# EternityJune25/ComoRAG

Hardware: AMD Instinct MI355X
Metric: top-k queries/sec (higher is better)
Workload: dtype bf16; 1 GPU; brute-force top-20 over 10000000 x 768 bf16 rows, batch 64, row-sharded over 1 GPU(s) (north_star target config); rows=10000000, dim=768, batch=64, k=20, query_batches_rotated=4, device=AMD Radeon Graphics (gfx950:sramecc+:xnack-), n_cu=256, repeats=1, exchange=none (1 shard)

## Files before the change

### comorag_amd/csrc/api.hip

```cpp
#include <hip/hip_runtime.h>

#include <algorithm>
#include <cmath>
#include <cstdarg>
#include <cstdio>
#include <cstdlib>
#include <cstring>
#include <chrono>
#include <atomic>
#include <climits>
#include <map>
#include <memory>
#include <mutex>
#include <shared_mutex>
#include <string>
#include <vector>

#include "../../include/comorag_hip.h"
#include "cmr_kernels.h"
#include "cmr_internal.h"
#include "index_state.h"
#include "search_plan.h"
#include "prefilter_host.h"

// ... 49 lines not shown
    {"sync_poll", OPT_FIELD(sync_poll), Option::any, 0, 0, 0, nullptr, nullptr},
    {"scan_fin_dense", OPT_FIELD(fin_dense), Option::clamp, 1, 1 << 16, 0, nullptr, nullptr},
    {"scan_fin_cap", OPT_FIELD(fin_cap), Option::oneof, 0, 128, 256, "scan_fin_cap must be 0, 128 or 256", nullptr},
    {"scan_fin_suppliers", OPT_FIELD(fin_suppliers), Option::clamp, 0, CMR_FIN_SLOTS / CMR_SCAN_WAVES, 0, nullptr, nullptr},
    {"scan_fin_spin", OPT_FIELD(fin_spin), Option::clamp, 0, 1000, 0, nullptr, nullptr},
    {"scan_fin_queries", OPT_FIELD(fin_max_q), Option::clamp, 1, CMR_FIN_MAX_QUERIES, 0, nullptr, nullptr},
    {"sample_div", OPT_FIELD(sample_div), Option::clamp, 2, LLONG_MAX, 0, nullptr, nullptr},
    {"sample_maxmul", OPT_FIELD(sample_maxmul), Option::clamp, 0, LLONG_MAX, 0, nullptr, nullptr},
    {"pipe_reserve_cus", OPT_FIELD(reserve_cus), Option::any, 0, 0, 0, nullptr, nullptr},
    {"pipe_slots", OPT_FIELD(pipe_slots), Option::any, 0, 0, 0, nullptr, nullptr},
    {"wide_mode", OPT_FIELD(wide_mode), Option::range, 0, 2, 0, "wide_mode must be 0 (default), 1 (register-resident kernel) or 2 (query-split grid)", nullptr},
    {"stream_nt", OPT_FIELD(stream_nt), Option::any, 0, 0, 0, nullptr, nullptr},
    {"pipe_dual_scan", OPT_FIELD(dual_scan), Option::any, 0, 0, 0, nullptr, nullptr},
    {"pipe_cu_mask", OPT_FIELD(cu_mask), Option::any, 0, 0, 0, nullptr, nullptr},
    {"exact_cand", OPT_FIELD(exact_cand), Option::range, 2, CMR_MAX_K, 0, "exact_cand must be in [2, " CMR_STR(CMR_MAX_K) "]", OPT_READ(i->exact_cand)},
    {"combine", [](cmr_index* i, long long v) { i->combine.store((int)v, std::memory_order_relaxed); }, Option::zero_or, 2, cmr_combine::kMaxWidth, 0,
     "combine must be 0 (off) or in [2, " CMR_STR(CMR_PPR_MAX_BATCH) "]", OPT_READ(i->combine.load(std::memory_order_relaxed))},
    {"combine_wait_us", [](cmr_index* i, long long v) { i->combine_wait_us.store(v, std::memory_order_relaxed); }, Option::clamp, 0, 10000000, 0, nullptr,
     OPT_READ(i->combine_wait_us.load(std::memory_order_relaxed))},
    {"prefilter", OPT_FIELD(prefilter), Option::range, -1, 2, 0, "prefilter must be -1 (auto), 0 (off), 1 (on) or 2 (on, the filter keeps every row)", OPT_READ(i->prefilter)},
    {"prefilter_rescore_wgs", OPT_FIELD(pf_rescore_wgs), Option::clamp, 0, 1024, 0, nullptr, nullptr},
    {"prefilter_tighten", OPT_FIELD(pf_tighten), Option::range, 0, 1, 0, "prefilter_tighten must be 0 or 1", OPT_READ(i->pf_tighten)},
    {"prefilter_pair_cap", OPT_FIELD(pf_pair_cap), Option::clamp, 0, 1 << 20, 0, nullptr, OPT_READ(i->pf_pair_cap)},
    {"prefilter_active", nullptr, Option::any, 0, 0, 0, nullptr, OPT_READ(i->prefilter_active)},
    {"prefilter_rows", nullptr, Option::any, 0, 0, 0, nullptr, OPT_READ(i->q8c.q8 ? i->q8c.rows : 0)},
    {"prefilter_bytes", nullptr, Option::any, 0, 0, 0, nullptr, OPT_READ((long long)i->q8c.bytes(i->dpad))},
    {"prefilter_candidates", nullptr, Option::any, 0, 0, 0, nullptr, OPT_READ(q8_read_counter(i, Q8Counter::candidates))},
    {"prefilter_pairs", nullptr, Option::any, 0, 0, 0, nullptr, OPT_READ(q8_read_counter(i, Q8Counter::pairs))},
    {"prefilter_pair_overflow", nullptr, Option::any, 0, 0, 0, nullptr, OPT_READ(q8_read_counter(i, Q8Counter::pair_overflow))},
    {"last_route", nullptr, Option::any, 0, 0, 0, nullptr, OPT_READ(i->last_route.load(std::memory_order_relaxed))},
    {"pipe_dual_scan_active", nullptr, Option::any, 0, 0, 0, nullptr, OPT_READ(i->dual_active)},
    {"pipe_dual_scan_wide_active", nullptr, Option::any, 0, 0, 0, nullptr, OPT_READ(i->dual_wide_active)},
    {"pipe_cu_mask_active", nullptr, Option::any, 0, 0, 0, nullptr, OPT_READ(i->pipe.last_masked)},
    {"pipe_scan_cus", nullptr, Option::any, 0, 0, 0, nullptr, OPT_READ(i->pipe.last_masked ? i->pipe.scan_cus : i->n_cu)},
    {"combine_batches", nullptr, Option::any, 0, 0, 0, nullptr, OPT_READ(i->combiner.batches())},
    {"combine_queries", nullptr, Option::any, 0, 0, 0, nullptr, OPT_READ(i->combiner.queries())},
    {"combine_max_width", nullptr, Option::any, 0, 0, 0, nullptr, OPT_READ(i->combiner.max_width())},
};
#undef OPT_FIELD
#undef OPT_READ

const Option* find_option(const char* name) {
    for (const Option& o : kOptions) if (strcmp(o.name, name) == 0) return &o;
    return nullptr;
}

int set_option(cmr_index* idx, const char* name, long long v) {
    const Option* o = find_option(name ? name : "");
    if (!o || !o->store) return fail(CMR_ERR_INVALID, "unknown option '%s'", name ? name : "");
    const bool refused = o->kind == Option::oneof ? (v != o->a && v != o->b && v != o->c) : o->kind == Option::range ? (v < o->a || v > o->b) : o->kind == Option::zero_or ? (v != 0 && (v < o->a || v > o->b)) : false;
    if (refused) return fail(CMR_ERR_INVALID, "%s", o->reject);
    if (o->kind == Option::clamp) v = std::max(o->a, std::min(v, o->b));
// ... 1555 lines not shown
```

### comorag_amd/csrc/cmr_kernels.h

```cpp
#pragma once
#include <hip/hip_runtime.h>
#include <stdint.h>

typedef unsigned long long u64;

struct CmrScanGeom {
    int dtype;
    int dpad;
    int ks;
    int nqt;
    int cap;
    int ring;
    int grid;
    int asm_ring;
    size_t lds;
    int stream_default_policy;
};

int cmr_scan_max_nqt(int dtype, int dpad);
bool cmr_scan_geom(CmrScanGeom* g);

struct CmrScanArgs {
    const void* corpus;
    const void* qfrag;
// ... 101 lines not shown
size_t cmr_exact_part_bytes(int nq, int kc);
hipError_t cmr_launch_exact_certify(int dtype, const float* shadow, int dim, long long nrows, long long id_base, const long long* tab, int nb,
                                    const float* q, int nq, const int64_t* cand_ids, const float* cand_sc, int kc, int k, const float* stats,
                                    void* part, int* arrive, int64_t* out_ids, float* out_scores, int* out_exact, hipStream_t s);

hipError_t cmr_launch_q8_quantise(int dtype, const void* corpus, int dpad, long long panel0, long long npanels, long long nrows, void* q8,
                                  float2* scales, float* stats, hipStream_t s);
hipError_t cmr_launch_q8_pack_queries(int dtype, const float* q, int nq, int dim, int dpad, int tiles, const float* stats, void* qpack,
                                      float4* qconst, hipStream_t s);
struct CmrQ8Args {
    int dtype, dpad, nqt, cap;
    int grid;
    int rescore_grid;
    const void* corpus;
    const void* q8;
    const float2* scales;
    const void* qfrag;
    const void* qpack;
    const float4* qconst;
    const u64* tau_init;
    long long nrows;
    int npanels, nq, k;
    int keep_all;
    void* pair;
    unsigned* pair_cnt;
    int pcap;
    unsigned* keep;
    float* tau_tight;
    unsigned* cand_row;
    unsigned* n_cand;
    u64* lists;
    int* cnt;
};
hipError_t cmr_launch_q8_filter(const CmrQ8Args& a, hipStream_t s);
hipError_t cmr_launch_q8_tighten(const CmrQ8Args& a, hipStream_t s);
hipError_t cmr_launch_q8_expand(const CmrQ8Args& a, hipStream_t s);
hipError_t cmr_launch_q8_rescore(const CmrQ8Args& a, hipStream_t s);
int cmr_q8_rescore_waves(void);
```

### comorag_amd/csrc/index_state.h

```cpp
#pragma once
#include <hip/hip_runtime.h>

#include <algorithm>
#include <atomic>
#include <cstring>
#include <map>
#include <mutex>
#include <shared_mutex>
#include <vector>

#include "../../include/comorag_hip.h"
#include "cmr_kernels.h"
#include "cmr_internal.h"
#include "combine.h"

#define CMR_DT_F32 0
#define CMR_PANEL_ROWS 32
#define CMR_SCAN_WAVES 8
#define CMR_CORPUS_SLACK (128 * 1024)

namespace {

int elem_size(int dtype) { return dtype == CMR_F32 ? 4 : 2; }
int round_up(int x, int m) { return (x + m - 1) / m * m; }
long long panels_of(long long rows) { return (rows + CMR_PANEL_ROWS - 1) / CMR_PANEL_ROWS; }

struct ExactScratch {
    DevBuf ids, sc, part, arrive, oids, osc, oex;
    void release() { ids.release(); sc.release(); part.release(); arrive.release(); oids.release(); osc.release(); oex.release(); }
};

struct Q8Companion {
    void* q8 = nullptr; float2* scales = nullptr; float* stats = nullptr;
    long long cap_panels = 0, rows = 0;
    long long failed_cap = -1;
    hipEvent_t ready = nullptr; hipStream_t stream = nullptr;
    size_t bytes(int dpad) const { return q8 ? (size_t)cap_panels * CMR_PANEL_ROWS * (dpad + sizeof(float2)) + CMR_CORPUS_SLACK : 0; }
    void release() { (void)hipFree(q8); (void)hipFree(scales); (void)hipFree(stats); if (ready) (void)hipEventDestroy(ready); *this = Q8Companion{}; }
};
enum Q8Buf { Q8_QPACK, Q8_QCONST, Q8_CAND, Q8_NCAND, Q8_PAIR, Q8_PAIRCNT, Q8_KEEP, Q8_TAU, Q8_NBUF };
struct Q8Scratch {
    DevBuf buf[Q8_NBUF];
    bool pf_prev = false;
    hipError_t ensure(const size_t (&bytes)[Q8_NBUF]) { for (int i = 0; i < Q8_NBUF; ++i) if (hipError_t e = buf[i].ensure(bytes[i])) return e; return hipSuccess; }
    void release() { for (DevBuf& b : buf) b.release(); }
};
struct Q8LastPass { const unsigned* ncand = nullptr; const unsigned* paircnt = nullptr; int nq = 0, pcap = 0; };

struct Workspace {
    hipStream_t stream = nullptr;
    bool own_stream = false;
    DevBuf qfrag, lists, cnt, mm, flag, tau, s_lists, s_cnt, s_mm, arrive;
    DevBuf fin_ctl, fin_pmax, fin_tau, fin_dense, fin_mm;
    bool fin_ctl_armed = false;
    DevBuf d_q, d_ids, d_scores, d_min, d_max, d_cand, d_out;
    DevBuf d_pack;
    Q8Scratch q8;
    ExactScratch x;
    int* flag_ptr = nullptr;
    int* done_ptr = nullptr;
    bool done_used = false;
    struct LazyMerge {
        bool due = false;
        const u64* lists = nullptr; const int* cnt = nullptr; int W = 0, NQ = 0, cap = 0, nqp = 0, k = 0; const float2* mm = nullptr; long long id_base = 0;
        int64_t* ids = nullptr; float* scores = nullptr; float* mn = nullptr; float* mx = nullptr; const int* state = nullptr;
    } lazy;
    void* h_pin = nullptr;
    void* h_pin_dev = nullptr;
    size_t h_pin_cap = 0;
    hipError_t ensure_pin(size_t need) {
// ... 81 lines not shown
    int sync_poll = 1;
    int scan_fin = 1;
    int fin_dense = 16384;
    int fin_cap = 0;
    int fin_suppliers = 0;
    int fin_spin = 0;
    int fin_max_q = 8;
    int dual_wide_active = 0;
    std::atomic<long long> last_route{0};
    int dual_active = 0;
    std::atomic<int> combine{0};
    std::atomic<long long> combine_wait_us{0};
    cmr_combine::Combiner combiner;
    long long id_base = 0;
    std::vector<long long> blk_local, blk_global;
    long long* d_blk = nullptr;
    std::vector<void*> blk_retired;
    int sample_maxmul = 0;
    int sample_div = 32;
    int prefilter = -1;
    int pf_rescore_wgs = 0;
    int pf_tighten = 1;
    int pf_pair_cap = 16384;
    Q8Companion q8c;
    int prefilter_active = 0;
    Q8LastPass q8_last;
    int pipe_slots = 3;
    int reserve_cus = -1;
    std::mutex pipe_mu;
    Pipe pipe;
    float* d_stats = nullptr;
    int exact_cand = CMR_MAX_K;
    ExactScratch x_slot[CMR_PIPE_SLOTS];
    unsigned x_next = 0;

    size_t panel_bytes() const { return (size_t)CMR_PANEL_ROWS * dpad * elem_size(dtype); }
    long long npanels() const { return panels_of(n); }
    int ks() const { return dtype == CMR_F32 ? dpad / 8 : dpad / 16; }
    int narrow_max() const { return cmr_scan_max_nqt(dtype, dpad) >= 2 ? 64 : 32; }
    int narrow_width(int nq) const { return nq > 32 ? narrow_max() : 32; }
    double scan_us() const { return (double)npanels() * panel_bytes() / 6.0e6; }
    bool short_scan() const { return scan_us() < 1000.0; }
    bool single_block() const { return blk_local.size() <= 1; }
    bool small_operands_fit() const { return (size_t)ks() * 1024 <= 143 * 1024; }
};

// ... 79 lines not shown
```

### comorag_amd/csrc/prefilter_host.h

```cpp
#pragma once
#include "search_plan.h"

namespace {

bool q8_ensure_companion(cmr_index* idx, hipStream_t s) {
    Q8Companion& c = idx->q8c;
    if (c.failed_cap == idx->cap_panels) return false;
    auto give_up = [&]() { c.release(); c.failed_cap = idx->cap_panels; (void)hipGetLastError(); return false; };
    if (c.q8 && c.cap_panels != idx->cap_panels) {
        if (hipDeviceSynchronize() != hipSuccess) return give_up();
        c.release();
    }
    if (!c.q8) {
        const size_t bytes = (size_t)idx->cap_panels * CMR_PANEL_ROWS * idx->dpad;
        if (hipMalloc((void**)&c.stats, 2 * sizeof(float)) != hipSuccess) { c.stats = nullptr; return give_up(); }
        if (hipEventCreateWithFlags(&c.ready, hipEventDisableTiming) != hipSuccess) { c.ready = nullptr; return give_up(); }
        if (hipMalloc(&c.q8, bytes + CMR_CORPUS_SLACK) != hipSuccess) { c.q8 = nullptr; return give_up(); }
        if (hipMalloc((void**)&c.scales, (size_t)idx->cap_panels * CMR_PANEL_ROWS * sizeof(float2)) != hipSuccess) { c.scales = nullptr; return give_up(); }
        if (hipMemsetAsync((char*)c.q8 + bytes, 0, CMR_CORPUS_SLACK, s) != hipSuccess || hipMemsetAsync(c.stats, 0, 2 * sizeof(float), s) != hipSuccess) return give_up();
        c.cap_panels = idx->cap_panels;
    }
    c.rows = std::min(c.rows, idx->n);
    if (c.rows < idx->n) {
        const long long panel0 = c.rows / CMR_PANEL_ROWS;
// ... 1 lines not shown
            hipEventRecord(c.ready, s) != hipSuccess) return give_up();
        c.stream = s; c.rows = idx->n;
    }
    return true;
}

constexpr bool kPrefilterAuto = true;
int prefilter_eligible(const cmr_index* idx, bool threshold, bool minmax, int nq, bool may_prefilter) {
    if (!may_prefilter || threshold || minmax || idx->dtype == CMR_F32 || idx->n <= 0 || nq > idx->narrow_max()) return 0;
    if (idx->prefilter < 0) return kPrefilterAuto && !idx->short_scan() ? 1 : 0;
    return idx->prefilter;
}

int q8_prepare(cmr_index* idx, Workspace* ws, const PassPlan& p, const float* q_dev, hipStream_t sp, CmrQ8Args& f) {
    const Q8Companion& c = idx->q8c;
    DevBuf* const w = ws->q8.buf;
    HIP_TRY(ws->q8.ensure(p.bytes.q8));
    if (sp != c.stream) HIP_TRY(hipStreamWaitEvent(sp, c.ready, 0));
    HIP_TRY(cmr_launch_q8_pack_queries(idx->dtype, q_dev, p.nqp, idx->dim, idx->dpad, p.tiles, c.stats, w[Q8_QPACK].p, (float4*)w[Q8_QCONST].p, sp));
    f.dtype = idx->dtype; f.dpad = idx->dpad; f.nqt = p.g.nqt; f.cap = p.g.cap; f.grid = p.g.grid; f.rescore_grid = p.rescore_grid;
    f.corpus = idx->corpus; f.q8 = c.q8; f.scales = c.scales; f.qfrag = ws->qfrag.p; f.qpack = w[Q8_QPACK].p; f.qconst = (const float4*)w[Q8_QCONST].p;
    f.nrows = idx->n; f.npanels = (int)idx->npanels(); f.nq = p.nqp; f.k = p.k; f.keep_all = p.prefilter == 2 ? 1 : 0;
    f.cand_row = (unsigned*)w[Q8_CAND].p; f.n_cand = (unsigned*)w[Q8_NCAND].p; f.keep = (unsigned*)w[Q8_KEEP].p; f.tau_tight = (float*)w[Q8_TAU].p;
    f.pair = w[Q8_PAIR].p; f.pair_cnt = (unsigned*)w[Q8_PAIRCNT].p; f.pcap = p.pair_cap;
    return CMR_OK;
}
int q8_filter(cmr_index* idx, CmrQ8Args& f, const CmrScanArgs& a, hipStream_t sm) {
    f.tau_init = a.tau_init; f.lists = a.lists; f.cnt = a.cnt;
    HIP_TRY(cmr_launch_q8_filter(f, sm));
    idx->q8_last = Q8LastPass{f.n_cand, f.pair_cnt, f.nq, f.pcap};
    idx->prefilter_active = 1;
    return CMR_OK;
}
int q8_rescore(const CmrQ8Args& f, hipStream_t sq) {
    if (f.pcap > 0) HIP_TRY(cmr_launch_q8_tighten(f, sq));
    HIP_TRY(hipMemsetAsync(f.n_cand, 0, sizeof(unsigned), sq));
    HIP_TRY(cmr_launch_q8_expand(f, sq));
    HIP_TRY(cmr_launch_q8_rescore(f, sq));
    return CMR_OK;
}
double prefilter_bytes(const cmr_index* idx, const PassPlan& p) {
    return (double)idx->npanels() * CMR_PANEL_ROWS * (idx->dpad + sizeof(float2)) + (double)2 * p.tiles * idx->dpad * 32;
}

enum class Q8Counter { candidates, pairs, pair_overflow };
long long q8_read_counter(const cmr_index* cidx, Q8Counter what) {
    cmr_index* idx = const_cast<cmr_index*>(cidx);
    if (cmr_set_device(idx->device)) return -1;
    std::lock_guard<std::mutex> pl(idx->pipe_mu);
    const Q8LastPass& L = idx->q8_last;
    const unsigned* const src = what == Q8Counter::candidates ? L.ncand : L.paircnt;
    std::vector<unsigned> h(what == Q8Counter::candidates ? 1 : (size_t)std::max(L.nq, 0));
    if (!src || h.empty()) return 0;
    for (hipStream_t st : idx->pipe.st) if (st && hipStreamSynchronize(st) != hipSuccess) return -1;
    if (hipMemcpy(h.data(), src, h.size() * sizeof(unsigned), hipMemcpyDeviceToHost) != hipSuccess) return -1;
    if (what == Q8Counter::candidates) return (long long)h[0];
    long long stored = 0, overflowed = 0;
    for (unsigned c : h) { stored += std::min(c, (unsigned)L.pcap); overflowed += c > (unsigned)L.pcap ? 1 : 0; }
    return what == Q8Counter::pairs ? stored : overflowed;
}

}
```

### comorag_amd/csrc/prefilter_kernels.hip

```cpp
#include "cmr_device.h"
#include "cmr_kernels.h"
#include "cmr_topk.h"

typedef __attribute__((ext_vector_type(16))) int i32x16;
typedef __attribute__((ext_vector_type(4))) int i32x4;

namespace {

template <int DT> __device__ __forceinline__ float q8_elem(unsigned short h) { return DT == CMR_DT_BF16 ? cmr_bf2f(h) : cmr_h2f(h); }
template <int DT> __device__ __forceinline__ unsigned short q8_round(float f) { return DT == CMR_DT_BF16 ? cmr_f2bf(f) : cmr_f2h(f); }

template <int DT> __device__ __forceinline__ void q8_unpack(const v4u& v, float (&x)[8]) {
    const unsigned w[4] = {v.x, v.y, v.z, v.w};
#pragma unroll
    for (int e = 0; e < 8; ++e) x[e] = q8_elem<DT>((unsigned short)(w[e >> 1] >> (16 * (e & 1))));
}

__device__ __forceinline__ float q8_up(double d) {
    float f = (float)d;
    if ((double)f < d) f = __uint_as_float(__float_as_uint(f) + 1u);
    return f;
}

__device__ __forceinline__ int q8_clamp(float v) { return (int)fminf(fmaxf(rintf(v), -127.0f), 127.0f); }
// ... 93 lines not shown
#pragma unroll
    for (int off = 32; off > 0; off >>= 1) { sQ += __shfl_xor(sQ, off); sf += __shfl_xor(sf, off); sq += __shfl_xor(sq, off); }
    if (lane == 0) { s_sum[0][wave] = sQ; s_sum[1][wave] = sf; s_sum[2][wave] = sq; }
    __syncthreads();
    if (tid == 0) {
        const double nQ = sqrt(s_sum[0][0] + s_sum[0][1] + s_sum[0][2] + s_sum[0][3]);
        const double nf = sqrt(s_sum[1][0] + s_sum[1][1] + s_sum[1][2] + s_sum[1][3]);
        const double nq2 = sqrt(s_sum[2][0] + s_sum[2][1] + s_sum[2][2] + s_sum[2][3]);
        const double Mx = (double)stats[0];
        const double gamma = (double)dpad * (1.0 / 8388608.0);
        const double c = (nf + gamma * nq2 + nQ * (1.0 / 1048576.0)) * Mx * (1.0 + 1e-5) + 1e-7;
        qconst[qi] = make_float4(a, q8_up(nQ * (1.0 + 1e-5)), q8_up(c), 0.0f);
    }
}

struct FilterP {
    const v4u* q8;
    const float4* scales4;
    const v4u* qpack;
    const float4* qconst;
    const u64* tau_init;
    long long nrows;
    int npanels, KB, nq, keep_all;
    v4u* pair;
    unsigned* pair_cnt;
    unsigned pcap;
    unsigned* keep;
};

template <int NQT, int CH>
__global__ __launch_bounds__(CMR_SCAN_THREADS, 1) void q8_filter_kernel(FilterP P) {
    extern __shared__ __attribute__((aligned(16))) unsigned char smem[];
    const int tid = threadIdx.x, lane = tid & 63;
    const int wave = __builtin_amdgcn_readfirstlane(tid >> 6);
    const int KB = P.KB;
    v4u* qf = reinterpret_cast<v4u*>(smem);
    for (int i = tid; i < 2 * NQT * KB * 64; i += CMR_SCAN_THREADS) qf[i] = P.qpack[i];
    __syncthreads();

    const int W = gridDim.x * CMR_SCAN_WAVES;
    const int gw = blockIdx.x * CMR_SCAN_WAVES + wave;
    const int p0 = (int)(((long long)gw * P.npanels) / W), p1 = (int)(((long long)(gw + 1) * P.npanels) / W);
    if (p1 <= p0) return;

    float aq[NQT], Bq[NQT], cq[NQT], tau[NQT];
    bool alive[NQT];
#pragma unroll
    for (int t = 0; t < NQT; ++t) {
        const int qi = t * 32 + (lane & 31);
        alive[t] = qi < P.nq;
        const float4 c = P.qconst[qi];
        aq[t] = c.x; Bq[t] = c.y; cq[t] = c.z;
        tau[t] = -__builtin_inff();
        if (alive[t] && P.tau_init && !P.keep_all) {
            const u64 key = P.tau_init[qi];
            if (key) tau[t] = cmr_key_score(key);
        }
    }

    i32x16 acc[2][NQT];
#pragma unroll
    for (int h = 0; h < 2; ++h)
#pragma unroll
        for (int t = 0; t < NQT; ++t)
#pragma unroll
            for (int r = 0; r < 16; ++r) acc[h][t][r] = 0;

    float4 sc[8];
    auto load_scales = [&](int p) {
        const float4* s = P.scales4 + (size_t)p * 16 + 2 * (lane >> 5);
#pragma unroll
        for (int g = 0; g < 4; ++g) { sc[2 * g] = s[4 * g]; sc[2 * g + 1] = s[4 * g + 1]; }
    };
    load_scales(p0);

    unsigned full = P.pcap ? 0u : ~0u;
    const int hrow = 4 * (lane >> 5);

    const int CPP = KB / CH;
    const long long nchunks = (long long)(p1 - p0) * CPP;
    const v4u* src = P.q8 + (size_t)p0 * KB * 64 + lane;
    int ci = 0, p = p0;
    v4u bufA[CH], bufB[CH];
    auto load = [&](v4u (&b)[CH]) {
#pragma unroll
        for (int u = 0; u < CH; ++u) b[u] = __builtin_nontemporal_load(&src[(size_t)u * 64]);
        src += (size_t)CH * 64;
    };
    auto step = [&](const v4u (&b)[CH]) {
        const v4u* qg = qf + (size_t)ci * CH * 64 + lane;
#pragma unroll
        for (int u = 0; u < CH; ++u) {
            const i32x4 a = __builtin_bit_cast(i32x4, b[u]);
#pragma unroll
            for (int t = 0; t < NQT; ++t) {
                acc[0][t] = __builtin_amdgcn_mfma_i32_32x32x32_i8(a, __builtin_bit_cast(i32x4, qg[((size_t)t * KB + u) * 64]), acc[0][t], 0, 0, 0);
                acc[1][t] = __builtin_amdgcn_mfma_i32_32x32x32_i8(a, __builtin_bit_cast(i32x4, qg[((size_t)(NQT + t) * KB + u) * 64]), acc[1][t], 0, 0, 0);
            }
        }
        if (++ci < CPP) return;
        ci = 0;
        unsigned hit = 0u;
#pragma unroll
        for (int r = 0; r < 16; ++r) {
            const float4 s4 = sc[2 * (r >> 2) + ((r & 3) >> 1)];
            const float ar = (r & 1) ? s4.z : s4.x, br = (r & 1) ? s4.w : s4.y;
#pragma unroll
            for (int t = 0; t < NQT; ++t) {
                const float ti = fmaf((float)acc[1][t][r], 1.0f / 254.0f, (float)acc[0][t][r]);
                const float ub = fmaf(ar * aq[t], ti, fmaf(Bq[t], br, cq[t]));
                if (alive[t] && !(ub < tau[t])) hit |= 1u << (r + 16 * t);
            }
        }
        const long long left = P.nrows - (long long)p * CMR_PANEL_ROWS;
        unsigned rows = 0u;
        if (P.keep_all) rows = ~0u;
        else if (__any(hit != 0u)) {
#pragma unroll
            for (int r = 0; r < 16; ++r) {
                const int i = (r & 3) + 8 * (r >> 2) + hrow;
                const float4 s4 = sc[2 * (r >> 2) + ((r & 3) >> 1)];
                const float ar = (r & 1) ? s4.z : s4.x, br = (r & 1) ? s4.w : s4.y;
#pragma unroll
                for (int t = 0; t < NQT; ++t) {
                    if (!(hit & (1u << (r + 16 * t))) || i >= left) continue;
                    if (full & (1u << t)) { rows |= 1u << i; continue; }
                    const int qi = t * 32 + (lane & 31);
                    const unsigned slot = atomicAdd(&P.pair_cnt[qi], 1u);
                    if (slot >= P.pcap) { full |= 1u << t; rows |= 1u << i; continue; }
                    const float ti = fmaf((float)acc[1][t][r], 1.0f / 254.0f, (float)acc[0][t][r]);
                    const float e = fmaf(Bq[t], br, cq[t]);
                    const float ub = fmaf(ar * aq[t], ti, e), lb = fmaf(ar * aq[t], ti, -e);
                    P.pair[(size_t)qi * P.pcap + slot] = (v4u){(unsigned)p * CMR_PANEL_ROWS + (unsigned)i, __float_as_uint(ub), __float_as_uint(lb), 0u};
                }
            }
#pragma unroll
            for (int off = 1; off < 64; off <<= 1) rows |= (unsigned)__shfl_xor((int)rows, off);
        }
        if (left < CMR_PANEL_ROWS) rows &= left > 0 ? (1u << left) - 1u : 0u;
        if (lane == 0) P.keep[p] = rows;
        ++p;
        load_scales(p < P.npanels ? p : P.npanels - 1);
#pragma unroll
        for (int h = 0; h < 2; ++h)
#pragma unroll
            for (int t = 0; t < NQT; ++t)
#pragma unroll
                for (int r = 0; r < 16; ++r) acc[h][t][r] = 0;
    };

    load(bufA);
    for (long long c = 0; c < nchunks; c += 2) {
        load(bufB);
        step(bufA);
        if (c + 1 < nchunks) {
            load(bufA);
            step(bufB);
        }
    }
}

struct TightenP {
    const v4u* pair;
    const unsigned* pair_cnt;
    unsigned pcap;
    const u64* tau_init;
    int k;
    unsigned* keep;
    float* tau_out;
};

__device__ __forceinline__ unsigned q8_f2ord(float f) { const unsigned u = __float_as_uint(f); return (u & 0x80000000u) ? ~u : (u | 0x80000000u); }
__device__ __forceinline__ float q8_ord2f(unsigned u) { return __uint_as_float((u & 0x80000000u) ? (u ^ 0x80000000u) : ~u); }

__global__ __launch_bounds__(256) void q8_tighten_kernel(TightenP P) {
    __shared__ unsigned hist[256];
    __shared__ unsigned s_bin, s_need;
    const int q = blockIdx.x, tid = threadIdx.x, lane = tid & 63;
    const unsigned offered = P.pair_cnt[q];
    const unsigned c = offered < P.pcap ? offered : P.pcap;
    const v4u* pr = P.pair + (size_t)q * P.pcap;
// ... 181 lines not shown
    }
    return hipGetLastError();
}

hipError_t cmr_launch_q8_pack_queries(int dtype, const float* q, int nq, int dim, int dpad, int tiles, const float* stats, void* qpack,
                                      float4* qconst, hipStream_t s) {
    const dim3 grid(tiles * 32), block(256);
    signed char* o = reinterpret_cast<signed char*>(qpack);
    switch (dtype) {
        case CMR_DT_BF16: hipLaunchKernelGGL(q8_pack_queries_kernel<CMR_DT_BF16>, grid, block, 0, s, q, nq, dim, dpad, tiles, stats, o, qconst); break;
        case CMR_DT_F16:  hipLaunchKernelGGL(q8_pack_queries_kernel<CMR_DT_F16>, grid, block, 0, s, q, nq, dim, dpad, tiles, stats, o, qconst); break;
        default: return hipErrorInvalidValue;
    }
    return hipGetLastError();
}

size_t cmr_q8_filter_lds(int dpad, int nqt) { return (size_t)2 * nqt * (dpad / 32) * 1024; }

hipError_t cmr_launch_q8_filter(const CmrQ8Args& a, hipStream_t s) {
    FilterP p;
    p.q8 = reinterpret_cast<const v4u*>(a.q8); p.scales4 = reinterpret_cast<const float4*>(a.scales);
    p.qpack = reinterpret_cast<const v4u*>(a.qpack); p.qconst = a.qconst; p.tau_init = a.tau_init;
    p.nrows = a.nrows; p.npanels = a.npanels; p.KB = a.dpad / 32; p.nq = a.nq; p.keep_all = a.keep_all;
    p.pair = reinterpret_cast<v4u*>(a.pair); p.pair_cnt = a.pair_cnt; p.pcap = a.keep_all ? 0u : (unsigned)a.pcap; p.keep = a.keep;
    const size_t lds = cmr_q8_filter_lds(a.dpad, a.nqt);
    auto launch = [&](auto kern) -> hipError_t {
        hipError_t e = hipFuncSetAttribute(reinterpret_cast<const void*>(kern), hipFuncAttributeMaxDynamicSharedMemorySize, 160 * 1024);
        if (e != hipSuccess) return e;
        hipLaunchKernelGGL(kern, dim3(a.grid), dim3(CMR_SCAN_THREADS), lds, s, p);
        return hipGetLastError();
    };
    const bool ch8 = p.KB % 8 == 0;
    if (a.nqt == 2) return ch8 ? launch(q8_filter_kernel<2, 8>) : launch(q8_filter_kernel<2, 4>);
    if (a.nqt == 1) return ch8 ? launch(q8_filter_kernel<1, 8>) : launch(q8_filter_kernel<1, 4>);
    return hipErrorInvalidValue;
}

hipError_t cmr_launch_q8_tighten(const CmrQ8Args& a, hipStream_t s) {
    TightenP p;
    p.pair = reinterpret_cast<const v4u*>(a.pair); p.pair_cnt = a.pair_cnt; p.pcap = (unsigned)a.pcap; p.tau_init = a.tau_init; p.k = a.k;
    p.keep = a.keep; p.tau_out = a.tau_tight;
    hipLaunchKernelGGL(q8_tighten_kernel, dim3(a.nq), dim3(256), 0, s, p);
    return hipGetLastError();
}

hipError_t cmr_launch_q8_expand(const CmrQ8Args& a, hipStream_t s) {
    hipLaunchKernelGGL(q8_expand_kernel, dim3((a.npanels + 255) / 256), dim3(256), 0, s, (const unsigned*)a.keep, a.npanels, a.cand_row, a.n_cand);
    return hipGetLastError();
}

hipError_t cmr_launch_q8_rescore(const CmrQ8Args& a, hipStream_t s) {
    RescoreP p;
    p.corpus = reinterpret_cast<const v4u*>(a.corpus); p.qfrag = reinterpret_cast<const v4u*>(a.qfrag);
    p.cand_row = a.cand_row; p.n_cand = a.n_cand; p.tau_init = a.tau_init; p.nrows = a.nrows; p.KS = a.dpad / 16; p.nq = a.nq; p.k = a.k;
    p.lists = a.lists; p.cnt = a.cnt;
    auto launch = [&](auto kern) -> hipError_t {
        hipLaunchKernelGGL(kern, dim3(a.rescore_grid), dim3(Q8_RESCORE_WAVES * 64), 0, s, p);
        return hipGetLastError();
// ... 9 lines not shown
```

### comorag_amd/csrc/search_plan.h

```cpp
#pragma once
#include <numeric>

#include "index_state.h"

bool cmr_ring_audit_ok(int dtype, int nqt, int cap, int ring, int mode);
static const long long kMaxMergeLists = 4096;

namespace {

int make_geom(const cmr_index* idx, int nq, int k, bool topk, CmrScanGeom* g) {
    const int max_nqt = cmr_scan_max_nqt(idx->dtype, idx->dpad);
    if (max_nqt == 0) return cmr_fail(CMR_ERR_UNSUPPORTED, "dim %d too large for the LDS-resident query tile (dtype %d)", idx->dim, idx->dtype);
    g->dtype = idx->dtype;
    g->dpad = idx->dpad;
    g->nqt = (nq > 32 && max_nqt >= 2) ? 2 : 1;
    g->cap = (topk && k > 32) ? 256 : 128;
    const int ks = idx->ks();
    g->ring = (ks % 16 == 0) ? 16 : 8;
    if (idx->force_ring == 8 || (idx->force_ring == 16 && ks % 16 == 0)) g->ring = idx->force_ring;
    const int mode = topk ? 0 : 1;
    g->asm_ring = cmr_ring_audit_ok(g->dtype, g->nqt, g->cap, g->ring, mode) ? 1 : 0;
    if (idx->force_asm == 0) g->asm_ring = 0;
    if (idx->force_asm == 1 && !cmr_ring_audit_ok(g->dtype, g->nqt, g->cap, g->ring, mode))
        return cmr_fail(CMR_ERR_UNSUPPORTED, "CMR_SCAN_ASM_RING=1 but variant (dtype %d nqt %d cap %d ring %d) failed the ISA audit", g->dtype, g->nqt, g->cap, g->ring);
// ... 22 lines not shown
}


enum class Route { narrow, wide, quad };

struct PassRequest {
    int nqp = 0, k = 0;
    Route route = Route::narrow;
    bool has_min_score = false;
    bool single_stream = false;
    bool pipelined = false;
    int reserve_cus = 0;
    int prefilter = 0;
};

struct PassPlan {
    int nqp = 0, k = 0;
    bool wide = false;
    CmrScanGeom g{};
    bool fin = false;
    int prefilter = 0;
    int rescore_grid = 0;
    int pair_cap = 0;
    int G = 1;
    int n_levels = 0;
    struct Level { long long panels; int grid, Wl, clog, stride; } level[2] = {};
    bool single_level = false;
    bool tau_in_scan = false;
    int reserve_cus = 0;
    int lists_per_wg = CMR_SCAN_WAVES;
    int NQ = 0, W = 0, Ws = 0, tiles = 0, NQA = 0;
    int fin_first = 0, fin_wgs = 0, fin_mul = 1, fin_dcap = 0, fin_spin = 0;
    struct { size_t qfrag, lists, cnt, mm, s_lists, s_cnt, s_mm, tau, fin_ctl, fin_pmax, fin_tau, fin_mm, fin_dense, q8[Q8_NBUF]; } bytes = {};
};

int plan_pass(const cmr_index* idx, const PassRequest& rq, PassPlan* out) {
    PassPlan& p = *out;
    p = PassPlan{};
    const int nqp = rq.nqp, k = rq.k;
    const bool wide = rq.route == Route::wide, quad = rq.route == Route::quad;
    p.nqp = nqp; p.k = k; p.wide = wide;
    CmrScanGeom& g = p.g;
    const long long npanels = idx->npanels();
    int rc = make_geom(idx, quad ? std::min(nqp, idx->narrow_max()) : nqp, k, true, &g);
    if (rc) return rc;
    const int G = quad ? (nqp + g.nqt * 32 - 1) / (g.nqt * 32) : 1;
// ... 58 lines not shown
        g.grid = (int)std::max<long long>(1, std::min<long long>(npanels, idx->n_cu));
        if (reserve_cus > 0 && g.grid > idx->n_cu / 2) g.grid = std::max(g.grid - reserve_cus, idx->n_cu / 2);
        NQ = nqb; W = g.grid; tiles = nqb / 32;
    } else if (G > 1) {
        if (reserve_cus > 0 && g.grid > idx->n_cu / 2) g.grid = std::max(g.grid - reserve_cus, idx->n_cu / 2);
        int vg = g.grid / G;
        if (vg >= 8) vg &= ~7;
        g.grid = std::max(vg, 1);
        NQ = g.nqt * 32; W = g.grid * CMR_SCAN_WAVES; tiles = G * g.nqt;
    } else {
        if (reserve_cus > 0 && g.grid > idx->n_cu / 2) g.grid = std::max(g.grid - reserve_cus, idx->n_cu / 2);
        if (!idx->force_grid) g.grid = balanced_grid(npanels, g.grid, CMR_SCAN_WAVES);
        NQ = g.nqt * 32; W = g.grid * CMR_SCAN_WAVES; tiles = g.nqt;
    }
    if (prefilter) {
        p.prefilter = rq.prefilter;
        p.rescore_grid = idx->pf_rescore_wgs > 0 ? idx->pf_rescore_wgs : std::min(idx->n_cu, 1024);
        W = p.rescore_grid * cmr_q8_rescore_waves();
        p.pair_cap = (rq.prefilter == 1 && idx->pf_tighten) ? idx->pf_pair_cap : 0;
        p.bytes.q8[Q8_QPACK] = (size_t)2 * tiles * (idx->dpad / 32) * 1024;
        p.bytes.q8[Q8_QCONST] = (size_t)NQ * sizeof(float4);
        p.bytes.q8[Q8_CAND] = (size_t)idx->cap_panels * CMR_PANEL_ROWS * sizeof(unsigned);
        p.bytes.q8[Q8_NCAND] = sizeof(unsigned);
        p.bytes.q8[Q8_PAIR] = std::max<size_t>((size_t)NQ * p.pair_cap * 16, 16);
        p.bytes.q8[Q8_PAIRCNT] = (size_t)NQ * sizeof(unsigned);
        p.bytes.q8[Q8_KEEP] = (size_t)idx->cap_panels * sizeof(unsigned);
        p.bytes.q8[Q8_TAU] = (size_t)NQ * sizeof(float);
    }
    const int NQA = G * NQ;
    p.NQ = NQ; p.W = W; p.Ws = Ws; p.tiles = tiles; p.NQA = NQA;
    p.bytes.qfrag = (size_t)tiles * g.ks * 1024;
    p.bytes.lists = (size_t)W * NQA * g.cap * 8;
    p.bytes.cnt = (size_t)W * NQA * 4;
    p.bytes.mm = (size_t)W * NQA * 8;
    p.bytes.s_lists = (size_t)Ws * NQA * g.cap * 8;
    p.bytes.s_cnt = (size_t)Ws * NQA * 4;
    p.bytes.s_mm = (size_t)Ws * NQA * 8;
    p.bytes.tau = (size_t)2 * NQA * 8;
    for (int lv = 0; lv < n_levels; ++lv) {
        PassPlan::Level& L = p.level[lv];
        const long long spn = level_panels[lv];
        L.panels = spn;
        L.grid = sample_grid(spn);
        L.Wl = L.grid * lists_per_wg;
        L.grid *= G;
        L.clog = spn >= 64 ? 3 : 0;
// ... 78 lines not shown
```

Baseline: 38460 queries/s.

## Buffer prefilter pairs per wave and bucket them by query in a separate kernel

The q8 filter kernel no longer does a global atomicAdd per (row, query) hit into per-query pair lists. Instead each wave appends records to its own buffer using ballot and mbcnt prefix offsets. A new bucket kernel then scatters these records into the per-query pair arrays, using LDS histograms and one global atomic per query per block. This aims to cut global atomic contention in the filter's hot loop, at the cost of an extra kernel launch, extra scratch memory, and a second pass over the records. Overflow falls back to keep bits via atomicOr. It also adds a sched_barrier after the loads and moves the tail masking earlier.

```diff
diff --git a/comorag_amd/csrc/api.hip b/comorag_amd/csrc/api.hip
--- a/comorag_amd/csrc/api.hip
+++ b/comorag_amd/csrc/api.hip
@@ -95,12 +95,14 @@
     {"prefilter_rescore_wgs", OPT_FIELD(pf_rescore_wgs), Option::clamp, 0, 1024, 0, nullptr, nullptr},
     {"prefilter_tighten", OPT_FIELD(pf_tighten), Option::range, 0, 1, 0, "prefilter_tighten must be 0 or 1", OPT_READ(i->pf_tighten)},
     {"prefilter_pair_cap", OPT_FIELD(pf_pair_cap), Option::clamp, 0, 1 << 20, 0, nullptr, OPT_READ(i->pf_pair_cap)},
+    {"prefilter_wave_cap", OPT_FIELD(pf_wave_cap), Option::clamp, 0, 1 << 20, 0, nullptr, OPT_READ(i->pf_wave_cap)},
     {"prefilter_active", nullptr, Option::any, 0, 0, 0, nullptr, OPT_READ(i->prefilter_active)},
     {"prefilter_rows", nullptr, Option::any, 0, 0, 0, nullptr, OPT_READ(i->q8c.q8 ? i->q8c.rows : 0)},
     {"prefilter_bytes", nullptr, Option::any, 0, 0, 0, nullptr, OPT_READ((long long)i->q8c.bytes(i->dpad))},
     {"prefilter_candidates", nullptr, Option::any, 0, 0, 0, nullptr, OPT_READ(q8_read_counter(i, Q8Counter::candidates))},
     {"prefilter_pairs", nullptr, Option::any, 0, 0, 0, nullptr, OPT_READ(q8_read_counter(i, Q8Counter::pairs))},
     {"prefilter_pair_overflow", nullptr, Option::any, 0, 0, 0, nullptr, OPT_READ(q8_read_counter(i, Q8Counter::pair_overflow))},
+    {"prefilter_wave_overflow", nullptr, Option::any, 0, 0, 0, nullptr, OPT_READ(q8_read_counter(i, Q8Counter::wave_overflow))},
     {"last_route", nullptr, Option::any, 0, 0, 0, nullptr, OPT_READ(i->last_route.load(std::memory_order_relaxed))},
     {"pipe_dual_scan_active", nullptr, Option::any, 0, 0, 0, nullptr, OPT_READ(i->dual_active)},
     {"pipe_dual_scan_wide_active", nullptr, Option::any, 0, 0, 0, nullptr, OPT_READ(i->dual_wide_active)},
diff --git a/comorag_amd/csrc/cmr_kernels.h b/comorag_amd/csrc/cmr_kernels.h
--- a/comorag_amd/csrc/cmr_kernels.h
+++ b/comorag_amd/csrc/cmr_kernels.h
@@ -147,6 +147,9 @@
     long long nrows;
     int npanels, nq, k;
     int keep_all;
+    void* wrec;
+    unsigned* wcnt;
+    int wave_cap;
     void* pair;
     unsigned* pair_cnt;
     int pcap;
@@ -158,6 +161,7 @@
     int* cnt;
 };
 hipError_t cmr_launch_q8_filter(const CmrQ8Args& a, hipStream_t s);
+hipError_t cmr_launch_q8_bucket(const CmrQ8Args& a, hipStream_t s);
 hipError_t cmr_launch_q8_tighten(const CmrQ8Args& a, hipStream_t s);
 hipError_t cmr_launch_q8_expand(const CmrQ8Args& a, hipStream_t s);
 hipError_t cmr_launch_q8_rescore(const CmrQ8Args& a, hipStream_t s);
diff --git a/comorag_amd/csrc/index_state.h b/comorag_amd/csrc/index_state.h
--- a/comorag_amd/csrc/index_state.h
+++ b/comorag_amd/csrc/index_state.h
@@ -38,14 +38,14 @@
     size_t bytes(int dpad) const { return q8 ? (size_t)cap_panels * CMR_PANEL_ROWS * (dpad + sizeof(float2)) + CMR_CORPUS_SLACK : 0; }
     void release() { (void)hipFree(q8); (void)hipFree(scales); (void)hipFree(stats); if (ready) (void)hipEventDestroy(ready); *this = Q8Companion{}; }
 };
-enum Q8Buf { Q8_QPACK, Q8_QCONST, Q8_CAND, Q8_NCAND, Q8_PAIR, Q8_PAIRCNT, Q8_KEEP, Q8_TAU, Q8_NBUF };
+enum Q8Buf { Q8_QPACK, Q8_QCONST, Q8_CAND, Q8_NCAND, Q8_WREC, Q8_WCNT, Q8_PAIR, Q8_PAIRCNT, Q8_KEEP, Q8_TAU, Q8_NBUF };
 struct Q8Scratch {
     DevBuf buf[Q8_NBUF];
     bool pf_prev = false;
     hipError_t ensure(const size_t (&bytes)[Q8_NBUF]) { for (int i = 0; i < Q8_NBUF; ++i) if (hipError_t e = buf[i].ensure(bytes[i])) return e; return hipSuccess; }
     void release() { for (DevBuf& b : buf) b.release(); }
 };
-struct Q8LastPass { const unsigned* ncand = nullptr; const unsigned* paircnt = nullptr; int nq = 0, pcap = 0; };
+struct Q8LastPass { const unsigned* ncand = nullptr; const unsigned* paircnt = nullptr; int nq = 0, pcap = 0; const unsigned* wcnt = nullptr; int nw = 0, wave_cap = 0; };
 
 struct Workspace {
     hipStream_t stream = nullptr;
@@ -173,6 +173,7 @@
     int pf_rescore_wgs = 0;
     int pf_tighten = 1;
     int pf_pair_cap = 16384;
+    int pf_wave_cap = 0;
     Q8Companion q8c;
     int prefilter_active = 0;
     Q8LastPass q8_last;
diff --git a/comorag_amd/csrc/prefilter_host.h b/comorag_amd/csrc/prefilter_host.h
--- a/comorag_amd/csrc/prefilter_host.h
+++ b/comorag_amd/csrc/prefilter_host.h
@@ -47,18 +47,22 @@
     f.corpus = idx->corpus; f.q8 = c.q8; f.scales = c.scales; f.qfrag = ws->qfrag.p; f.qpack = w[Q8_QPACK].p; f.qconst = (const float4*)w[Q8_QCONST].p;
     f.nrows = idx->n; f.npanels = (int)idx->npanels(); f.nq = p.nqp; f.k = p.k; f.keep_all = p.prefilter == 2 ? 1 : 0;
     f.cand_row = (unsigned*)w[Q8_CAND].p; f.n_cand = (unsigned*)w[Q8_NCAND].p; f.keep = (unsigned*)w[Q8_KEEP].p; f.tau_tight = (float*)w[Q8_TAU].p;
+    f.wrec = w[Q8_WREC].p; f.wcnt = (unsigned*)w[Q8_WCNT].p; f.wave_cap = f.keep_all ? 0 : p.wave_cap;
     f.pair = w[Q8_PAIR].p; f.pair_cnt = (unsigned*)w[Q8_PAIRCNT].p; f.pcap = p.pair_cap;
     return CMR_OK;
 }
 int q8_filter(cmr_index* idx, CmrQ8Args& f, const CmrScanArgs& a, hipStream_t sm) {
     f.tau_init = a.tau_init; f.lists = a.lists; f.cnt = a.cnt;
     HIP_TRY(cmr_launch_q8_filter(f, sm));
-    idx->q8_last = Q8LastPass{f.n_cand, f.pair_cnt, f.nq, f.pcap};
+    idx->q8_last = Q8LastPass{f.n_cand, f.pair_cnt, f.nq, f.pcap, f.wcnt, f.grid * CMR_SCAN_WAVES, f.wave_cap};
     idx->prefilter_active = 1;
     return CMR_OK;
 }
 int q8_rescore(const CmrQ8Args& f, hipStream_t sq) {
-    if (f.pcap > 0) HIP_TRY(cmr_launch_q8_tighten(f, sq));
+    if (f.pcap > 0) {
+        HIP_TRY(cmr_launch_q8_bucket(f, sq));
+        HIP_TRY(cmr_launch_q8_tighten(f, sq));
+    }
     HIP_TRY(hipMemsetAsync(f.n_cand, 0, sizeof(unsigned), sq));
     HIP_TRY(cmr_launch_q8_expand(f, sq));
     HIP_TRY(cmr_launch_q8_rescore(f, sq));
@@ -68,18 +72,19 @@
     return (double)idx->npanels() * CMR_PANEL_ROWS * (idx->dpad + sizeof(float2)) + (double)2 * p.tiles * idx->dpad * 32;
 }
 
-enum class Q8Counter { candidates, pairs, pair_overflow };
+enum class Q8Counter { candidates, pairs, pair_overflow, wave_overflow };
 long long q8_read_counter(const cmr_index* cidx, Q8Counter what) {
     cmr_index* idx = const_cast<cmr_index*>(cidx);
     if (cmr_set_device(idx->device)) return -1;
     std::lock_guard<std::mutex> pl(idx->pipe_mu);
     const Q8LastPass& L = idx->q8_last;
-    const unsigned* const src = what == Q8Counter::candidates ? L.ncand : L.paircnt;
-    std::vector<unsigned> h(what == Q8Counter::candidates ? 1 : (size_t)std::max(L.nq, 0));
+    const unsigned* const src = what == Q8Counter::candidates ? L.ncand : what == Q8Counter::wave_overflow ? L.wcnt : L.paircnt;
+    std::vector<unsigned> h(what == Q8Counter::candidates ? 1 : (size_t)std::max(what == Q8Counter::wave_overflow ? (L.wave_cap > 0 ? L.nw : 0) : L.nq, 0));
     if (!src || h.empty()) return 0;
     for (hipStream_t st : idx->pipe.st) if (st && hipStreamSynchronize(st) != hipSuccess) return -1;
     if (hipMemcpy(h.data(), src, h.size() * sizeof(unsigned), hipMemcpyDeviceToHost) != hipSuccess) return -1;
     if (what == Q8Counter::candidates) return (long long)h[0];
+    if (what == Q8Counter::wave_overflow) return (long long)std::count_if(h.begin(), h.end(), [&](unsigned c) { return c > (unsigned)L.wave_cap; });
     long long stored = 0, overflowed = 0;
     for (unsigned c : h) { stored += std::min(c, (unsigned)L.pcap); overflowed += c > (unsigned)L.pcap ? 1 : 0; }
     return what == Q8Counter::pairs ? stored : overflowed;
diff --git a/comorag_amd/csrc/prefilter_kernels.hip b/comorag_amd/csrc/prefilter_kernels.hip
--- a/comorag_amd/csrc/prefilter_kernels.hip
+++ b/comorag_amd/csrc/prefilter_kernels.hip
@@ -139,9 +139,9 @@
     const u64* tau_init;
     long long nrows;
     int npanels, KB, nq, keep_all;
-    v4u* pair;
-    unsigned* pair_cnt;
-    unsigned pcap;
+    v4u* wrec;
+    unsigned* wcnt;
+    unsigned wave_cap;
     unsigned* keep;
 };
 
@@ -158,7 +158,10 @@
     const int W = gridDim.x * CMR_SCAN_WAVES;
     const int gw = blockIdx.x * CMR_SCAN_WAVES + wave;
     const int p0 = (int)(((long long)gw * P.npanels) / W), p1 = (int)(((long long)(gw + 1) * P.npanels) / W);
-    if (p1 <= p0) return;
+    if (p1 <= p0) {
+        if (lane == 0) P.wcnt[gw] = 0u;
+        return;
+    }
 
     float aq[NQT], Bq[NQT], cq[NQT], tau[NQT];
     bool alive[NQT];
@@ -191,7 +194,8 @@
     };
     load_scales(p0);
 
-    unsigned full = P.pcap ? 0u : ~0u;
+    v4u* const wr = P.wrec + (size_t)gw * P.wave_cap;
+    unsigned nrec = 0u;
     const int hrow = 4 * (lane >> 5);
 
     const int CPP = KB / CH;
@@ -203,6 +207,7 @@
 #pragma unroll
         for (int u = 0; u < CH; ++u) b[u] = __builtin_nontemporal_load(&src[(size_t)u * 64]);
         src += (size_t)CH * 64;
+        __builtin_amdgcn_sched_barrier(0);
     };
     auto step = [&](const v4u (&b)[CH]) {
         const v4u* qg = qf + (size_t)ci * CH * 64 + lane;
@@ -230,31 +235,46 @@
             }
         }
         const long long left = P.nrows - (long long)p * CMR_PANEL_ROWS;
+        if (left < CMR_PANEL_ROWS) {
+            const int lim = (int)(left > 0 ? left : 0) - hrow;
+#pragma unroll
+            for (int r = 0; r < 16; ++r)
+                if ((r & 3) + 8 * (r >> 2) >= lim) hit &= ~(0x10001u << r);
+        }
         unsigned rows = 0u;
-        if (P.keep_all) rows = ~0u;
+        if (P.keep_all) rows = left < CMR_PANEL_ROWS ? (left > 0 ? (1u << left) - 1u : 0u) : ~0u;
         else if (__any(hit != 0u)) {
-#pragma unroll
-            for (int r = 0; r < 16; ++r) {
-                const int i = (r & 3) + 8 * (r >> 2) + hrow;
-                const float4 s4 = sc[2 * (r >> 2) + ((r & 3) >> 1)];
-                const float ar = (r & 1) ? s4.z : s4.x, br = (r & 1) ? s4.w : s4.y;
-#pragma unroll
-                for (int t = 0; t < NQT; ++t) {
-                    if (!(hit & (1u << (r + 16 * t))) || i >= left) continue;
-                    if (full & (1u << t)) { rows |= 1u << i; continue; }
-                    const int qi = t * 32 + (lane & 31);
-                    const unsigned slot = atomicAdd(&P.pair_cnt[qi], 1u);
-                    if (slot >= P.pcap) { full |= 1u << t; rows |= 1u << i; continue; }
-                    const float ti = fmaf((float)acc[1][t][r], 1.0f / 254.0f, (float)acc[0][t][r]);
-                    const float e = fmaf(Bq[t], br, cq[t]);
-                    const float ub = fmaf(ar * aq[t], ti, e), lb = fmaf(ar * aq[t], ti, -e);
-                    P.pair[(size_t)qi * P.pcap + slot] = (v4u){(unsigned)p * CMR_PANEL_ROWS + (unsigned)i, __float_as_uint(ub), __float_as_uint(lb), 0u};
+            const unsigned row0 = (unsigned)p * CMR_PANEL_ROWS + (unsigned)hrow;
+            if (P.wave_cap == 0u) {
+#pragma unroll
+                for (int r = 0; r < 16; ++r)
+                    if (hit & (0x10001u << r)) rows |= 1u << ((r & 3) + 8 * (r >> 2));
+            } else {
+#pragma unroll
+                for (int r = 0; r < 16; ++r) {
+                    const float4 s4 = sc[2 * (r >> 2) + ((r & 3) >> 1)];
+                    const float ar = (r & 1) ? s4.z : s4.x, br = (r & 1) ? s4.w : s4.y;
+#pragma unroll
+                    for (int t = 0; t < NQT; ++t) {
+                        const bool h = (hit & (1u << (r + 16 * t))) != 0u;
+                        const u64 m = __ballot(h);
+                        if (m == 0ull) continue;
+                        const unsigned slot = nrec + __builtin_amdgcn_mbcnt_hi((unsigned)(m >> 32), __builtin_amdgcn_mbcnt_lo((unsigned)m, 0u));
+                        nrec += (unsigned)__popcll(m);
+                        if (!h) continue;
+                        if (slot >= P.wave_cap) { rows |= 1u << ((r & 3) + 8 * (r >> 2)); continue; }
+                        const float ti = fmaf((float)acc[1][t][r], 1.0f / 254.0f, (float)acc[0][t][r]);
+                        const float e = fmaf(Bq[t], br, cq[t]);
+                        const float ub = fmaf(ar * aq[t], ti, e), lb = fmaf(ar * aq[t], ti, -e);
+                        wr[slot] = (v4u){row0 + (unsigned)((r & 3) + 8 * (r >> 2)), __float_as_uint(ub), __float_as_uint(lb),
+                                         (unsigned)(t * 32 + (lane & 31))};
+                    }
                 }
             }
+            rows <<= hrow;
 #pragma unroll
             for (int off = 1; off < 64; off <<= 1) rows |= (unsigned)__shfl_xor((int)rows, off);
         }
-        if (left < CMR_PANEL_ROWS) rows &= left > 0 ? (1u << left) - 1u : 0u;
         if (lane == 0) P.keep[p] = rows;
         ++p;
         load_scales(p < P.npanels ? p : P.npanels - 1);
@@ -274,6 +294,45 @@
             load(bufA);
             step(bufB);
         }
+    }
+    if (lane == 0) P.wcnt[gw] = nrec;
+}
+
+struct BucketP {
+    const v4u* wrec;
+    const unsigned* wcnt;
+    unsigned wave_cap;
+    int W;
+    v4u* pair;
+    unsigned* pair_cnt;
+    unsigned pcap;
+    unsigned* keep;
+};
+
+#define Q8_BUCKET_WAVES 4
+__global__ __launch_bounds__(Q8_BUCKET_WAVES * 64) void q8_bucket_kernel(BucketP P) {
+    __shared__ unsigned s_cnt[64], s_base[64];
+    const int tid = threadIdx.x, lane = tid & 63;
+    const int w = blockIdx.x * Q8_BUCKET_WAVES + (tid >> 6);
+    if (tid < 64) s_cnt[tid] = 0u;
+    __syncthreads();
+    unsigned c = 0u;
+    if (w < P.W) { const unsigned offered = P.wcnt[w]; c = offered < P.wave_cap ? offered : P.wave_cap; }
+    const v4u* rec = P.wrec + (size_t)(w < P.W ? w : 0) * P.wave_cap;
+    for (unsigned i = lane; i < c; i += 64u) atomicAdd(&s_cnt[rec[i].w & 63u], 1u);
+    __syncthreads();
+    if (tid < 64) {
+        const unsigned n = s_cnt[tid];
+        s_base[tid] = n ? atomicAdd(&P.pair_cnt[tid], n) : 0u;
+        s_cnt[tid] = 0u;
+    }
+    __syncthreads();
+    for (unsigned i = lane; i < c; i += 64u) {
+        const v4u v = rec[i];
+        const unsigned q = v.w & 63u;
+        const unsigned slot = s_base[q] + atomicAdd(&s_cnt[q], 1u);
+        if (slot < P.pcap) P.pair[(size_t)q * P.pcap + slot] = (v4u){v.x, v.y, v.z, 0u};
+        else atomicOr(&P.keep[v.x >> 5], 1u << (v.x & 31u));
     }
 }
 
@@ -501,7 +560,7 @@
     p.q8 = reinterpret_cast<const v4u*>(a.q8); p.scales4 = reinterpret_cast<const float4*>(a.scales);
     p.qpack = reinterpret_cast<const v4u*>(a.qpack); p.qconst = a.qconst; p.tau_init = a.tau_init;
     p.nrows = a.nrows; p.npanels = a.npanels; p.KB = a.dpad / 32; p.nq = a.nq; p.keep_all = a.keep_all;
-    p.pair = reinterpret_cast<v4u*>(a.pair); p.pair_cnt = a.pair_cnt; p.pcap = a.keep_all ? 0u : (unsigned)a.pcap; p.keep = a.keep;
+    p.wrec = reinterpret_cast<v4u*>(a.wrec); p.wcnt = a.wcnt; p.wave_cap = (unsigned)a.wave_cap; p.keep = a.keep;
     const size_t lds = cmr_q8_filter_lds(a.dpad, a.nqt);
     auto launch = [&](auto kern) -> hipError_t {
         hipError_t e = hipFuncSetAttribute(reinterpret_cast<const void*>(kern), hipFuncAttributeMaxDynamicSharedMemorySize, 160 * 1024);
@@ -513,6 +572,14 @@
     if (a.nqt == 2) return ch8 ? launch(q8_filter_kernel<2, 8>) : launch(q8_filter_kernel<2, 4>);
     if (a.nqt == 1) return ch8 ? launch(q8_filter_kernel<1, 8>) : launch(q8_filter_kernel<1, 4>);
     return hipErrorInvalidValue;
+}
+
+hipError_t cmr_launch_q8_bucket(const CmrQ8Args& a, hipStream_t s) {
+    BucketP p;
+    p.wrec = reinterpret_cast<const v4u*>(a.wrec); p.wcnt = a.wcnt; p.wave_cap = (unsigned)a.wave_cap; p.W = a.grid * CMR_SCAN_WAVES;
+    p.pair = reinterpret_cast<v4u*>(a.pair); p.pair_cnt = a.pair_cnt; p.pcap = (unsigned)a.pcap; p.keep = a.keep;
+    hipLaunchKernelGGL(q8_bucket_kernel, dim3((p.W + Q8_BUCKET_WAVES - 1) / Q8_BUCKET_WAVES), dim3(Q8_BUCKET_WAVES * 64), 0, s, p);
+    return hipGetLastError();
 }
 
 hipError_t cmr_launch_q8_tighten(const CmrQ8Args& a, hipStream_t s) {
diff --git a/comorag_amd/csrc/search_plan.h b/comorag_amd/csrc/search_plan.h
--- a/comorag_amd/csrc/search_plan.h
+++ b/comorag_amd/csrc/search_plan.h
@@ -68,6 +68,7 @@
     int prefilter = 0;
     int rescore_grid = 0;
     int pair_cap = 0;
+    int wave_cap = 0;
     int G = 1;
     int n_levels = 0;
     struct Level { long long panels; int grid, Wl, clog, stride; } level[2] = {};
@@ -172,6 +173,10 @@
         p.bytes.q8[Q8_QCONST] = (size_t)NQ * sizeof(float4);
         p.bytes.q8[Q8_CAND] = (size_t)idx->cap_panels * CMR_PANEL_ROWS * sizeof(unsigned);
         p.bytes.q8[Q8_NCAND] = sizeof(unsigned);
+        const long long fw = (long long)g.grid * CMR_SCAN_WAVES;
+        p.wave_cap = !p.pair_cap ? 0 : idx->pf_wave_cap > 0 ? idx->pf_wave_cap : (int)std::min<long long>(1 << 20, (((long long)NQ * p.pair_cap + fw - 1) / fw + 63) / 64 * 64);
+        p.bytes.q8[Q8_WREC] = std::max<size_t>((size_t)fw * p.wave_cap * 16, 16);
+        p.bytes.q8[Q8_WCNT] = (size_t)fw * sizeof(unsigned);
         p.bytes.q8[Q8_PAIR] = std::max<size_t>((size_t)NQ * p.pair_cap * 16, 16);
         p.bytes.q8[Q8_PAIRCNT] = (size_t)NQ * sizeof(unsigned);
         p.bytes.q8[Q8_KEEP] = (size_t)idx->cap_panels * sizeof(unsigned);
```

After: 41430 queries/s, median of 6. 1.08x the previous value.
